# DeepLearnPhysics/u-resnet

Measured on AMD Instinct MI355X. Metric: fwd+bwd images/sec on 3D 192^3x1 U-ResNet, higher is better.
Workload: dtype f32

## Files before the change

### u-resnet_amd/csrc/conv_tiled.hip

```cpp
#include <stdlib.h>

#include "conv_tiled_kernel.h"
#include "wgrad_tiled_kernel.h"

int twgradq_dispatch(const TWPlan& p, const TWgradArgs& a, hipStream_t s);
int twgrad4_dispatch_3d(const TWPlan& p, const TWgradArgs& a, hipStream_t s);
int twgrad4_dispatch_2d(const TWPlan& p, const TWgradArgs& a, hipStream_t s);
int twgradz_dispatch(const TWPlan& p, const TWgradArgs& a, hipStream_t s);

static bool tiled_shape_ok(int cin, int cout, int mode) {
  if (cin % 4 || cout % 4 || cin < 4 || cout < 4) return false;
  if ((cin == 8 || cin == 16) && (cout == 8 || cout == 16)) return true;
  if (mode == 3) return (cin == 8 && cout == 4) || (cin == 4 && cout == 8);
  return (cin == 32 && cout == 16) || (cin == 16 && cout == 32) || (cin == 16 && cout == 4) || (cin == 4 && cout == 16) ||
         (cin == 4 && cout == 8);
}

static bool tiled_disabled() {
  static int v = -1;
  if (v < 0) { const char* e = getenv("URSN_DISABLE_TILED"); v = (e && e[0] == '1') ? 1 : 0; }
  return v == 1;
}

struct Blocking {
// ... 372 lines not shown
      URSN_TRY(launch_reduce_accum_blocked(dw + (size_t)8 * bi * 8, (const float*)scratch, taps, 8, 8, (int64_t)d.cin * 8,
                                           8, nslab, s));
    }
    return 0;
  }
  if (!blocked && use_wgrad4(d, p)) {
    a.x = x;
    a.dz = dy;
    URSN_TRY(p.mode == 3 ? twgrad4_dispatch_3d(p, a, s) : twgrad4_dispatch_2d(p, a, s));
    return launch_reduce_accum(dw, (const float*)scratch, (int64_t)taps * d.cin * d.cout, p.grid, s);
  }
  for (int bi = 0; bi < b.nbi; ++bi)
    for (int bo = 0; bo < b.nbo; ++bo) {
      a.x = x + 16 * bi;
      a.dz = dy + 16 * bo;
      URSN_TRY(p.mode == 3 ? twgrad_dispatch_3d(p, a, s) : twgrad_dispatch_2d(p, a, s));
      if (!blocked) return launch_reduce_accum(dw, (const float*)scratch, (int64_t)taps * d.cin * d.cout, p.grid, s);
      URSN_TRY(launch_reduce_accum_blocked(dw + (size_t)16 * bi * d.cout + 16 * bo, (const float*)scratch, taps, 16, 16,
                                           (int64_t)d.cin * d.cout, d.cout, p.grid, s));
    }
  ursn_relabel_kernel("twgrad<16,16>xB");
  return 0;
}
```

### u-resnet_amd/csrc/elementwise.hip

```cpp
#include "ursn_common.h"

typedef float f32x4 __attribute__((ext_vector_type(4)));

static int next_pow2(int x) { int p = 1; while (p < x) p <<= 1; return p; }

template <int VEC> struct VT;
template <> struct VT<1> { typedef float T; };
template <> struct VT<4> { typedef f32x4 T; };

#ifndef URSN_EW_NT
#define URSN_EW_NT 1
#endif
#ifndef URSN_EW_U
#define URSN_EW_U 2
#endif
#ifndef URSN_EW_ACT_U
#define URSN_EW_ACT_U 4
#endif
template <int VEC> __device__ inline typename VT<VEC>::T ldv(const float* p) {
#if URSN_EW_NT & 1
  return __builtin_nontemporal_load((const typename VT<VEC>::T*)p);
#else
  return *(const typename VT<VEC>::T*)p;
#endif
// ... 305 lines not shown
}

__global__ __launch_bounds__(256) void bn_bwd_final_kernel(const double* __restrict__ partial, int nblocks, int C,
                                                           int64_t V, double* __restrict__ finals,
                                                           float* __restrict__ dbeta, float* __restrict__ dbeta2, int Cw,
                                                           float* __restrict__ coef, const float* __restrict__ mean,
                                                           const float* __restrict__ rstd, const float* __restrict__ beta) {
  const int c = blockIdx.x;
  double s[3];
  reduce_partials<3>(partial, nblocks, C, c, s);
  if (threadIdx.x != 0) return;
  finals[c] = s[0] / (double)V;
  finals[C + c] = s[1] / (double)V;
  finals[2 * C + c] = s[2] / (double)V;
  if (coef) {
    const float r = rstd[c], mu = mean[c];
    const float mg = (float)finals[c], mgx = (float)finals[C + c];
    coef[c] = r;
    coef[C + c] = -(r * r) * mgx;
    coef[2 * C + c] = -r * mg;
    coef[3 * C + c] = mu;
    coef[4 * C + c] = r;
    coef[5 * C + c] = beta ? beta[c] - mu * r : 0.f;
  }
  if (c >= Cw) return;
  if (dbeta) dbeta[c] += (float)s[0];
  if (dbeta2) dbeta2[c] += (float)s[0];
}

template <int VEC>
__global__ __launch_bounds__(256) void bn_bwd_apply_kernel(BnBwdArgs a, int shift, const double* __restrict__ finals) {
  const int CP = 1 << shift;
  const int VPB = 256 >> shift;
  const int c = (threadIdx.x & (CP - 1)) * VEC;
  const int vr = threadIdx.x >> shift;
  if (c >= a.C) return;
  float mu[VEC], rs[VEC], mu2[VEC], rs2[VEC], mg[VEC], mgx[VEC], mgx2[VEC], be[VEC];
  const bool bmask = VEC == 4 && a.relu && a.mask != nullptr;
  const bool ymask = !bmask && a.relu && a.y != nullptr, zmask = !bmask && a.relu && a.y == nullptr;
  const int lane = threadIdx.x & 63;
#pragma unroll
  for (int j = 0; j < VEC; ++j) {
    mu[j] = a.mean[c + j];
    rs[j] = a.rstd[c + j];
    be[j] = zmask ? a.beta[c + j] - mu[j] * rs[j] : 0.f;
    mu2[j] = a.z2 ? a.mean2[c + j] : 0.f;
// ... 68 lines not shown
  Map m = make_map(a.V, a.C, v4 ? 4 : 1);
  double* partial = (double*)a.scratch;
  double* finals = partial + (size_t)m.grid * 3 * a.C;
  int nblocks = m.grid;
  if (a.pre_partial) {
    partial = const_cast<double*>(a.pre_partial);
    nblocks = a.pre_nblocks;
  } else {
    if (v4) hipLaunchKernelGGL(bn_bwd_reduce_kernel<4>, dim3(m.grid), dim3(256), 0, s, a, m.shift, partial);
    else hipLaunchKernelGGL(bn_bwd_reduce_kernel<1>, dim3(m.grid), dim3(256), 0, s, a, m.shift, partial);
    URSN_HIP(hipGetLastError());
  }
  if (a.coef_out) URSN_REQUIRE(!a.z2 && !a.dres && !a.mask && !(a.relu && a.y), "bn_bwd: apply-on-load coefficients need a single BatchNorm, no residual share and the bn(z) > 0 mask");
  hipLaunchKernelGGL(bn_bwd_final_kernel, dim3(a.C), dim3(256), 0, s, (const double*)partial, nblocks, a.C, a.V, finals,
                     a.dbeta, a.z2 ? a.dbeta2 : nullptr, a.Cw > 0 ? a.Cw : a.C, a.coef_out, a.mean, a.rstd, a.relu ? a.beta : nullptr);
  URSN_HIP(hipGetLastError());
  if (a.coef_out) return 0;
  if (v4) hipLaunchKernelGGL(bn_bwd_apply_kernel<4>, dim3(m.grid), dim3(256), 0, s, a, m.shift, (const double*)finals);
  else hipLaunchKernelGGL(bn_bwd_apply_kernel<1>, dim3(m.grid), dim3(256), 0, s, a, m.shift, (const double*)finals);
  URSN_HIP(hipGetLastError());
  return 0;
}

#define URSN_MAX_CLASS 8
__global__ __launch_bounds__(256) void head_kernel(HeadArgs a, double* __restrict__ partial) {
  const int64_t P = (int64_t)a.n * a.pix;
  double loss = 0.0;
  unsigned int n_ok = 0, n_nz = 0, n_ok_nz = 0;
  float sc[URSN_MAX_CLASS], sh[URSN_MAX_CLASS];
#pragma unroll
  for (int k = 0; k < URSN_MAX_CLASS; ++k) {
    sc[k] = 1.f;
    sh[k] = 0.f;
    if (k < a.ncls && a.mean) {
      sc[k] = a.rstd[k];
      sh[k] = a.beta[k] - a.mean[k] * sc[k];
    }
  }
  const float invn = 1.0f / (float)a.n;
  float bg[4] = {0.f, 0.f, 0.f, 0.f}, bgx[4] = {0.f, 0.f, 0.f, 0.f};
  float mu[4];
#pragma unroll
  for (int k = 0; k < 4; ++k) mu[k] = (k < a.ncls && a.mean) ? a.mean[k] : 0.f;
  for (int64_t p = (int64_t)blockIdx.x * blockDim.x + threadIdx.x; p < P; p += (int64_t)gridDim.x * blockDim.x) {
    float z[URSN_MAX_CLASS];
    float m = -INFINITY;
// ... 293 lines not shown
```

### u-resnet_amd/csrc/net.hip

```cpp
#include <math.h>
#include <stdio.h>
#include <stdlib.h>
#include <string.h>

#include <map>
#include <string>
#include <vector>

#include "ursn_common.h"
#include "net_bf16.h"

int conv_dispatch(const ursn_conv_desc& d, ConvPass pass, const float* in, const float* w, float* out, int accumulate,
                  hipStream_t s);
int wgrad_dispatch(const ursn_conv_desc& d, const float* x, const float* dy, float* dw, void* scratch,
                   size_t scratch_bytes, hipStream_t s);

namespace {

struct Arena {
  char* base = nullptr;
  size_t off = 0;
  void* take(size_t bytes) {
    off = (off + 255) & ~(size_t)255;
    void* p = base ? (void*)(base + off) : nullptr;
// ... 43 lines not shown
  int ldim[8][3];
  int64_t lvox[8];
  std::vector<Layer> layers;
  std::vector<Unit> units;
  std::vector<int> deconv;
  std::vector<Act> deconv_in, deconv_out, cat;
  int conv0 = -1, conv1 = -1, conv2 = -1;
  Act a_data, a_conv0, a_conv1, a_pre1;
  std::vector<int> ginit;
  float *params = nullptr, *grads = nullptr, *adam_m = nullptr, *adam_v = nullptr;
  float* dlog = nullptr;
  float* metrics = nullptr;
  void* red_scratch = nullptr;
  void* red_scratch2 = nullptr;
  void* head_scratch = nullptr;
  void* wg_scratch = nullptr;
  size_t wg_scratch_bytes = 0;
  float* dc_scratch = nullptr;
  double* bs_scratch = nullptr;
  int bs_layer = -1, bs_blocks = 0;
  int bs_C = 8;
  int vdz_layer = -1, vdz_relu = 0, vdz_cs = 0;
  const float* vdz_g = nullptr;
  int64_t adam_t = 0;
  int last_n = 0;
  bool profile = false;
  struct ProfRec { int layer; int pass; const char* kernel; double flops; double bytes; hipEvent_t e0, e1; long l0; int launches; };
  std::vector<ProfRec> prof;
  std::vector<hipEvent_t> ev_pool;
  size_t ev_used = 0;
  hipStream_t s2 = nullptr;
  hipStream_t s2_owned = nullptr;
  struct StepGraph { const float* data; const float* label; const float* weight; int n, seen; hipGraphExec_t exec; };
  std::vector<StepGraph> graphs;
  bool graph_broken = false;
  hipStream_t gstream = nullptr;
  hipEvent_t g_in = nullptr, g_out = nullptr;
  std::vector<hipEvent_t> sync_pool;
  size_t sync_used = 0;
  std::vector<hipEvent_t> fwd_pool;
  size_t fwd_used = 0;
  hipEvent_t s2_done = nullptr;
  std::vector<std::pair<std::string, std::string>> cat_names;
  std::map<std::string, Act> named;
  std::map<std::string, int> named_z;
};
// ... 28 lines not shown
int add_layer(ursn_net* n, Arena& A, const std::string& name, int kind, int k, int s, int ci, int co, int lin, int lout,
              int64_t& poff, int relu = 0) {
  Layer L;
  L.name = "UResNet/" + name;
  L.relu = relu;
  L.kind = kind; L.k = k; L.stride = s; L.cin = ci; L.cout = co; L.lin = lin; L.lout = lout;
  int64_t taps = 1;
  for (int j = 0; j < n->cfg.ndim; ++j) taps *= k;
  L.w_n = taps * ci * co;
  L.w_off = poff; poff += L.w_n;
  L.b_off = poff; poff += co;
  memset(&L.desc, 0, sizeof(L.desc));
  L.desc.ndim = n->cfg.ndim;
  L.desc.n = n->cfg.max_batch;
  for (int j = 0; j < n->cfg.ndim; ++j) L.desc.in_sp[j] = n->ldim[lin][3 - n->cfg.ndim + j];
  L.desc.cin = ci; L.desc.cout = co; L.desc.k = k; L.desc.stride = s; L.desc.transposed = kind;
  L.zcs = (co + 3) & ~3;
  L.desc.out_cstride = L.zcs;
  int64_t e = (int64_t)n->cfg.max_batch * n->lvox[lout] * L.zcs;
  L.z = A.floats(e);
  L.dz = n->cfg.trainable ? A.floats(e) : nullptr;
  L.mean = A.floats(L.zcs);
  L.rstd = A.floats(L.zcs);
  L.coef = n->cfg.trainable ? A.floats(6 * L.zcs) : nullptr;
  n->layers.push_back(L);
  n->named_z[L.name] = (int)n->layers.size() - 1;
  return (int)n->layers.size() - 1;
}

int plan(ursn_net* n, Arena& A) {
  const ursn_config& c = n->cfg;
  URSN_REQUIRE(c.ndim == 2 || c.ndim == 3, "len(dims) must be 3 (H,W,C) or 4 (H,W,D,C)");
  URSN_REQUIRE(c.num_strides >= 1 && c.num_strides <= 5, "num_strides %d out of range [1,5]", c.num_strides);
  URSN_REQUIRE(c.cin >= 1 && c.base_filters >= 1 && c.num_class >= 1 && c.num_class <= 8 && c.max_batch >= 1,
               "bad channel / class / batch configuration");
  const int ns = c.num_strides;
  n->nlev = ns + 1;
  for (int l = 0; l <= ns; ++l) {
    n->lvox[l] = 1;
    for (int j = 0; j < 3; ++j) {
      int lead = 3 - c.ndim;
      if (j < lead) { n->ldim[l][j] = 1; continue; }
      int s0 = c.spatial[j - lead];
      URSN_REQUIRE(s0 > 0 && s0 % (1 << ns) == 0, "spatial size %d not divisible by 2^%d (deconv/skip shapes would differ)", s0, ns);
      n->ldim[l][j] = s0 >> l;
      n->lvox[l] *= n->ldim[l][j];
    }
// ... 463 lines not shown
      if (blocks > 0 && blocks <= 16384 && tiled_conv_supported(u, PASS_DGRAD)) { t = u; n->bs_layer = bs->li; n->bs_blocks = blocks; }
    }
    {
      ProfScope pd(n, s, li, 1, 2.0 * layer_macs(n, L, N), layer_bytes(n, L, N));
      URSN_TRY(conv_dispatch(t, PASS_DGRAD, n->vdz_g, n->params + L.w_off, in.g, acc ? 1 : 0, s));
      pd.done(ursn_last_kernel_name());
    }
    need_dgrad = false;
  }
  hipStream_t ws = s;
  if (n->s2) {
    if (n->sync_used == n->sync_pool.size()) {
      hipEvent_t e;
      URSN_HIP(hipEventCreateWithFlags(&e, hipEventDisableTiming));
      n->sync_pool.push_back(e);
    }
    hipEvent_t e = n->sync_pool[n->sync_used++];
    URSN_HIP(hipEventRecord(e, s));
    URSN_HIP(hipStreamWaitEvent(n->s2, e, 0));
    ws = n->s2;
  }
  {
    ProfScope ps(n, ws, li, 2, 2.0 * layer_macs(n, L, N), layer_bytes(n, L, N));
    URSN_TRY(wgrad_dispatch(d, in.p, L.dz, n->grads + L.w_off, n->wg_scratch, n->wg_scratch_bytes, ws));
    ps.done(ursn_last_kernel_name());
  }
  if (dgrad_done_elsewhere) {
    ProfScope pd(n, s, li, 1, 2.0 * layer_macs(n, L, N), layer_bytes(n, L, N));
    pd.done("(fused into conv1 dgrad)");
  }
  if (need_dgrad) {
    bool acc = take_flag(n, in);
    if (in2) URSN_REQUIRE(take_flag(n, *in2) == acc, "split input: the two halves disagree on gradient initialisation");
    d = bwd_desc(n, li, in, N, in2, fused_sc);
    n->bs_layer = -1;
    static const bool bs_off = getenv("URSN_FUSE_BN_BWD_REDUCE") && getenv("URSN_FUSE_BN_BWD_REDUCE")[0] == '0';
    if (bs && bs->li >= 0 && !bs_off) {
      const Layer& T = n->layers[bs->li];
      ursn_conv_desc t = d;
      t.bs_z = T.z; t.bs_z_cstride = T.zcs; t.bs_mean = T.mean; t.bs_rstd = T.rstd; t.bs_beta = n->params + T.b_off;
      t.bs_relu = bs->relu; t.bs_mask = bs->mask;
      if (bs->li2 >= 0) {
        const Layer& T2 = n->layers[bs->li2];
        t.bs_z2 = T2.z; t.bs_z2_cstride = T2.zcs; t.bs_mean2 = T2.mean; t.bs_rstd2 = T2.rstd;
      }
      t.bs_partial = n->bs_scratch;
      const bool fits = T.cout == 8 && T.zcs == 8 && in.C == 8 && in.cs == 8 && !in2 &&
// ... 3 lines not shown
    }
    ProfScope pd(n, s, li, 1, 2.0 * layer_macs(n, L, N), layer_bytes(n, L, N));
    if (n->dc_scratch && deep_conv_supported(d, PASS_DGRAD))
      URSN_TRY(launch_deep_conv(d, PASS_DGRAD, L.dz, n->params + L.w_off, in.g, acc ? 1 : 0, n->dc_scratch, nullptr, 0.f, nullptr, nullptr, s));
    else
      URSN_TRY(conv_dispatch(d, PASS_DGRAD, L.dz, n->params + L.w_off, in.g, acc ? 1 : 0, s));
    pd.done(ursn_last_kernel_name());
  }
  return 0;
}

bool vdz_ok(ursn_net* n, int li, const Act& in, int N, bool two_z_target) {
  static const int mode = getenv("URSN_FUSE_BN_BWD_APPLY") ? atoi(getenv("URSN_FUSE_BN_BWD_APPLY")) : 1;
  const bool off = mode == 0 || (mode == 1 && two_z_target);
  const Layer& L = n->layers[li];
  if (off || n->cfg.ndim != 3 || L.kind || L.k != 3 || L.stride != 1 || L.cin != 8 || L.cout != 8 || L.zcs != 8 || in.C != 8 || in.cs != 8 || !in.g)
    return false;
  ursn_conv_desc d = L.desc;
  d.n = N; d.in_cstride = in.cs; d.out_cstride = L.zcs;
  d.vdz_z = L.z; d.vdz_coef = L.coef; d.vdz_out = L.dz;
  return tiled_conv_supported(d, PASS_DGRAD) != 0;
}

int bn_back(ursn_net* n, int li, const float* dy, int dycs, const float* y, int ycs, int relu, int li2, float* dres,
            int drescs, int dres_acc, int N, hipStream_t s, const unsigned long long* mask = nullptr, const Act* fuse_in = nullptr,
            bool fuse_two_z = false) {
  Layer& L = n->layers[li];
  BnBwdArgs a;
  memset(&a, 0, sizeof(a));
  a.dy = dy; a.dycs = dycs; a.y = mask ? nullptr : y; a.ycs = ycs; a.mask = mask;
  a.z = L.z; a.zcs = L.zcs; a.mean = L.mean; a.rstd = L.rstd; a.dz = L.dz; a.dzcs = L.zcs;
  a.dbeta = n->grads + L.b_off;
  a.beta = n->params + L.b_off;
  if (li2 >= 0) {
    Layer& L2 = n->layers[li2];
    a.z2 = L2.z; a.z2cs = L2.cout; a.mean2 = L2.mean; a.rstd2 = L2.rstd; a.dz2 = L2.dz; a.dz2cs = L2.cout;
    a.dbeta2 = n->grads + L2.b_off;
  }
  a.dres = dres; a.drescs = drescs; a.dres_accumulate = dres_acc;
  a.V = (int64_t)N * n->lvox[L.lout]; a.C = L.cout; a.relu = relu; a.scratch = n->red_scratch;
  if (L.zcs != L.cout && li2 < 0 && !relu && dycs == L.zcs && !dres) { a.C = L.zcs; a.Cw = L.cout; }
  if (n->bs_layer == li && a.C == n->bs_C) { a.pre_partial = n->bs_scratch; a.pre_nblocks = n->bs_blocks; }
  n->bs_layer = -1;
  n->bs_C = 8;
  n->vdz_layer = -1;
  if (fuse_in && li2 < 0 && !dres && !mask && !y && dycs == L.zcs && vdz_ok(n, li, *fuse_in, N, fuse_two_z)) {
    a.coef_out = L.coef;
    n->vdz_layer = li; n->vdz_relu = relu; n->vdz_g = dy; n->vdz_cs = dycs;
  }
  ProfScope ps(n, s, li, 5, 0.0, 4.0 * a.V * a.C * (2.0 * (2 + (relu && !mask) + (li2 >= 0)) + 1 + (li2 >= 0) + (dres != nullptr)));
  URSN_TRY(launch_bn_bwd(a, s));
  ps.done("bn_bwd");
  return 0;
}

int unit_bwd(ursn_net* n, Unit& u, int N, hipStream_t s, const BsTarget* in_target = nullptr) {
  if (u.sc >= 0) {
    URSN_TRY(bn_back(n, u.c2, u.out.g, u.out.cs, u.out.p, u.out.cs, 1, u.sc, nullptr, 0, 0, N, s, u.jmask));
  } else {
    bool acc = take_flag(n, u.in);
    URSN_TRY(bn_back(n, u.c2, u.out.g, u.out.cs, u.out.p, u.out.cs, 1, -1, u.in.g, u.in.cs, acc ? 1 : 0, N, s, u.jmask));
  }
  BsTarget t1;
  t1.li = u.c1;
  if (u.a1_virtual) {
    Act z1 = u.a1;
    z1.p = n->layers[u.c1].z; z1.cs = n->layers[u.c1].zcs;
    URSN_TRY(conv_bwd(n, u.c2, z1, true, N, s, nullptr, -1, false, u.c1, &t1));
  } else {
    URSN_TRY(conv_bwd(n, u.c2, u.a1, true, N, s, nullptr, -1, false, -1, &t1));
  }
  URSN_TRY(bn_back(n, u.c1, u.a1.g, u.a1.cs, nullptr, 0, 0, -1, nullptr, 0, 0, N, s, nullptr, (u.in2.C || u.sc >= 0) ? nullptr : &u.in,
                   in_target && in_target->li2 >= 0));
// ... 34 lines not shown
    if (u.jmask) { t.li = u.c2; t.li2 = u.sc; t.relu = 2; t.mask = u.jmask; }
    return t;
  };
  auto act_of = [&](int li) { BsTarget t; t.li = li; t.relu = 1; return t; };
  tc = join_of(n->units[ui - 1]);
  URSN_TRY(conv_bwd(n, n->conv1, n->a_pre1, true, N, s, nullptr, -1, false, -1, &tc));
  for (int i = ns - 1; i >= 0; --i) {
    tc = join_of(n->units[ui - 2]);
    URSN_TRY(unit_bwd(n, n->units[--ui], N, s, &tc));
    tc = act_of(n->deconv[i]);
    URSN_TRY(unit_bwd(n, n->units[--ui], N, s, &tc));
    const Act& dout = n->deconv_out[i];
    URSN_TRY(bn_back(n, n->deconv[i], dout.g, dout.cs, nullptr, 0, 1, -1, nullptr, 0, 0, N, s));
    tc = join_of(n->units[ui - 1]);
    URSN_TRY(conv_bwd(n, n->deconv[i], n->deconv_in[i], true, N, s, nullptr, -1, false, -1, &tc));
  }
  for (int step = ns - 1; step >= 0; --step) {
    tc = join_of(n->units[ui - 2]);
    URSN_TRY(unit_bwd(n, n->units[--ui], N, s, &tc));
    tc = ui >= 2 ? join_of(n->units[ui - 2]) : act_of(n->conv0);
    URSN_TRY(unit_bwd(n, n->units[--ui], N, s, &tc));
  }
  const Act& a0 = n->a_conv0;
  URSN_TRY(bn_back(n, n->conv0, a0.g, a0.cs, nullptr, 0, 1, -1, nullptr, 0, 0, N, s));
  Act din = n->a_data;
  din.p = const_cast<float*>(data);
  URSN_TRY(conv_bwd(n, n->conv0, din, false, N, s));
  if (n->s2) {
    URSN_HIP(hipEventRecord(n->s2_done, n->s2));
    URSN_HIP(hipStreamWaitEvent(s, n->s2_done, 0));
  }
  return 0;
}

int read_metrics(ursn_net* n, float* out, int cnt, hipStream_t s) {
  float h[4];
  URSN_HIP(hipMemcpyAsync(h, n->metrics, sizeof(h), hipMemcpyDeviceToHost, s));
  URSN_HIP(hipStreamSynchronize(s));
  if (cnt == 3) { out[0] = h[0]; out[1] = h[1]; out[2] = h[2]; }
  else { out[0] = h[1]; out[1] = h[2]; }
  return 0;
}

int check_call(ursn_net* n, const float* data, int N) {
  URSN_REQUIRE(n, "null handle");
  URSN_REQUIRE(data, "input_data is null");
  URSN_REQUIRE(N >= 1 && N <= n->cfg.max_batch, "batch %d outside [1,%d]", N, n->cfg.max_batch);
  return 0;
}
// ... 320 lines not shown
  std::string s(name);
  bool want_z = false, want_g = false, want_dz = false, want_mean = false, want_rstd = false;
  auto strip = [&](const char* suf, bool& f) {
    size_t L = strlen(suf);
    if (s.size() > L && s.compare(s.size() - L, L, suf) == 0) { f = true; s = s.substr(0, s.size() - L); }
  };
  strip(":dz", want_dz);
  strip(":z", want_z);
  strip(":grad", want_g);
  strip(":mean", want_mean);
  strip(":rstd", want_rstd);
  if (want_g && s == "logits") {
    URSN_REQUIRE(net->dlog, "tensor: net is not trainable");
    const Layer& L = net->layers[net->conv2];
    *ptr = net->dlog; *voxels = net->lvox[0]; *channels = L.cout; *cstride = L.zcs;
    return 0;
  }
  if (want_z || want_dz || want_mean || want_rstd) {
    auto it = net->named_z.find(s);
    URSN_REQUIRE(it != net->named_z.end(), "tensor: no layer named %s", s.c_str());
    const Layer& L = net->layers[it->second];
    *ptr = want_z ? L.z : want_dz ? L.dz : want_mean ? L.mean : L.rstd;
    URSN_REQUIRE(*ptr, "tensor: %s does not exist (net is not trainable)", name);
    *voxels = (want_mean || want_rstd) ? 0 : net->lvox[L.lout];
    *channels = L.cout;
    *cstride = L.zcs;
    return 0;
  }
  auto it = net->named.find(s);
  URSN_REQUIRE(it != net->named.end(), "tensor: no activation named %s", s.c_str());
  *ptr = want_g ? it->second.g : it->second.p;
  URSN_REQUIRE(*ptr, "tensor: %s is not materialised (normalised on load inside the consuming convolution, URSN_NORM_ON_LOAD=1)", name);
  *voxels = net->lvox[it->second.lvl];
  *channels = it->second.C;
  *cstride = it->second.cs;
  return 0;
}

extern "C" int ursn_profile_enable(ursn_net* net, int32_t on) {
  URSN_REQUIRE(net, "null handle");
  if (net->bf) return bnet_profile_enable(net->bf, on);
  net->profile = on != 0;
  net->prof.clear();
  net->ev_used = 0;
  return 0;
}
// ... 31 lines not shown
```

### u-resnet_amd/csrc/ursn_common.h

```cpp
#pragma once
#include <hip/hip_runtime.h>
#include <stdint.h>
#include <stddef.h>

#include "../../include/uresnet_hip.h"

void ursn_set_error(const char* fmt, ...);
void ursn_note_kernel(const char* name);
void ursn_relabel_kernel(const char* name);
#ifdef __HIPCC__
#ifndef URSN_XCD_REMAP
#define URSN_XCD_REMAP 1
#endif
__device__ __forceinline__ int ursn_xcd_block(int b, int G) {
#if URSN_XCD_REMAP
  const int q = G >> 3, r = G & 7, x = b & 7, i = b >> 3;
  return (x < r ? x * (q + 1) : r * (q + 1) + (x - r) * q) + i;
#else
  return b;
#endif
}

__device__ __forceinline__ void ursn_sacc(float piv, float& s1, float& s2, float v) {
  const float d = v - piv;
// ... 71 lines not shown
enum ConvPass { PASS_FWD = 0, PASS_DGRAD = 1, PASS_WGRAD = 2 };
int build_geoms(const ursn_conv_desc& d, ConvPass pass, GatherGeom* out8);

struct BnStats {
  double* sum;
  float* mean;
  float* rstd;
};

size_t reduce_scratch_bytes(int64_t voxels, int channels, int nsums);
int reduce_nblocks(int64_t voxels, int channels);

int launch_bn_stats(const float* z, int zcs, int64_t V, int C, float eps, float* mean, float* rstd,
                    void* scratch, hipStream_t s);
int launch_bn_stats_final(const double* partial, int nblocks, int C, int PC, int64_t V, float eps, float* mean,
                          float* rstd, hipStream_t s);
int launch_bn_stats_final_blocked(const double* partial, int nblocks, int C, int CB, int PC, size_t blk_stride, int64_t V, float eps,
                                  float* mean, float* rstd, hipStream_t s);
int tiled_conv_supported(const ursn_conv_desc& d, ConvPass pass);
size_t tiled_conv_stats_scratch_doubles(const ursn_conv_desc& d);
int launch_tiled_conv_bn(const ursn_conv_desc& d, const float* in, const float* w, float* out, double* scratch,
                         float eps, float* mean, float* rstd, hipStream_t s);
int tiled_wgrad_supported(const ursn_conv_desc& d);
int tiled_conv_bs_blocks(const ursn_conv_desc& d);
int igemm_conv_supported(const ursn_conv_desc& d, ConvPass pass);
size_t igemm_stats_scratch_doubles(const ursn_conv_desc& d);
int launch_igemm_conv(const ursn_conv_desc& d, ConvPass pass, const float* in, const float* w, float* out,
                      int accumulate, double* stats_partial, float eps, float* mean, float* rstd, hipStream_t s);
int igemm_wgrad_supported(const ursn_conv_desc& d);
size_t igemm_wgrad_scratch_bytes(const ursn_conv_desc& d);
int launch_igemm_wgrad(const ursn_conv_desc& d, const float* x, const float* dy, float* dw, void* scratch,
                       size_t scratch_bytes, hipStream_t s);
int deep_conv_supported(const ursn_conv_desc& d, ConvPass pass);
size_t deep_conv_scratch_floats(const ursn_conv_desc& d, ConvPass pass);
size_t deep_conv_stats_scratch_doubles(const ursn_conv_desc& d);
int launch_deep_conv(const ursn_conv_desc& d, ConvPass pass, const float* in, const float* w, float* out, int accumulate,
                     float* scratch, double* stats_partial, float eps, float* mean, float* rstd, hipStream_t s);
int deep_wgrad_supported(const ursn_conv_desc& d);
size_t deep_wgrad_scratch_bytes(const ursn_conv_desc& d);
int launch_deep_wgrad(const ursn_conv_desc& d, const float* x, const float* dy, float* dw, void* scratch, size_t scratch_bytes,
                      hipStream_t s);
int pointwise_conv_supported(const ursn_conv_desc& d, ConvPass pass, int accumulate);
size_t pointwise_stats_scratch_doubles(const ursn_conv_desc& d);
int launch_pointwise_conv(const ursn_conv_desc& d, ConvPass pass, const float* in, const float* w, float* out,
                          int accumulate, double* stats_partial, float eps, float* mean, float* rstd, hipStream_t s);
int pointwise_wgrad_supported(const ursn_conv_desc& d);
// ... 30 lines not shown
  const float* res; int rescs;
  float* y; int ycs;
  int64_t V; int C; int relu;
  unsigned long long* mask_out;
};
int launch_bn_act(const BnActArgs& a, hipStream_t s);
static inline size_t bn_mask_words(int64_t V, int C) { return (size_t)((V * C + 255) / 256) * 4; }
static inline bool bn_mask_ok(int C) { int q = C / 4; return (C % 4) == 0 && q >= 1 && q <= 64 && (q & (q - 1)) == 0; }

struct BnBwdArgs {
  const float* dy; int dycs; const float* y; int ycs;
  const float* z; int zcs; const float* mean; const float* rstd; float* dz; int dzcs; float* dbeta;
  const float* beta;
  const float* z2; int z2cs; const float* mean2; const float* rstd2; float* dz2; int dz2cs; float* dbeta2;
  float* dres; int drescs; int dres_accumulate;
  int64_t V; int C; int relu;
  void* scratch;
  const unsigned long long* mask;
  const double* pre_partial; int pre_nblocks;
  int Cw;
  float* coef_out;
};
int launch_bn_bwd(const BnBwdArgs& a, hipStream_t s);

struct HeadArgs {
  const float* z; int z_cs; const float* mean; const float* rstd; const float* beta;
  const float* data; int data_cs; const float* label; const float* weight;
  int n; int64_t pix; int ncls;
  float* softmax_out; float* dlogits;
  int dl_cs;
  float* ana_out;
  double* partial;
  float* metrics;
  void* scratch;
  double* bs_partial;
};
size_t head_scratch_bytes(int n, int64_t pix);
int head_blocks(int n, int64_t pix);
int launch_head_final(const double* partial, int nblocks, int n, int64_t pix, float* metrics, hipStream_t s);
int launch_bn_bwd_final(const double* partial, int nblocks, int C, int64_t V, double* finals, float* dbeta, float* dbeta2,
                        int Cw, hipStream_t s, float* coef_out = nullptr, const float* mean = nullptr, const float* rstd = nullptr,
                        const float* beta = nullptr);
int launch_head(const HeadArgs& a, hipStream_t s);

int launch_adam(float* p, const float* g, float* m, float* v, int64_t n, float lr_t, float b1, float b2,
                float eps, hipStream_t s);
// ... 4 lines not shown
```

### u-resnet_amd/csrc/wgrad_tiled_3d.hip

```cpp
#include "wgrad_tiled_kernel.h"

int twgrad_dispatch_3d(const TWPlan& p, const TWgradArgs& a, hipStream_t s) {
  constexpr int MODE = 3;
  URSN_TW(8, 8) URSN_TW(16, 8) URSN_TW(8, 16) URSN_TW(16, 16) URSN_TW(8, 4) URSN_TW(1, 8)
  ursn_set_error("tiled wgrad 3d: no instantiation for %d->%d", p.cin, p.cout);
  return 3;
}
```

### u-resnet_amd/csrc/wgrad_tiled_kernel.h

```cpp
#pragma once
#include <utility>

#include "ursn_common.h"
#include "buffer_stage.h"

typedef float wg_f32x4 __attribute__((ext_vector_type(4)));

struct TWgradArgs {
  const float* x;
  const float* dz;
  float* slab;
  int N, Z, Y, X;
  int x_cs, dz_cs;
  int zseg, nzseg, nty, ntx;
  int cout_w;
  const float* aff_mean;
  const float* aff_rstd;
  const float* aff_beta;
};

template <int MODE> struct WTile;
template <> struct WTile<3> { static constexpr int TX = 32, TY = 8, NTY = 3, NT = 27; };
template <> struct WTile<2> { static constexpr int TX = 256, TY = 1, NTY = 1, NT = 9; };

template <int... Is, class F>
__device__ __forceinline__ void wg_static_for_impl(std::integer_sequence<int, Is...>, F&& f) {
  (f(std::integral_constant<int, Is>{}), ...);
}
template <int N, class F>
__device__ __forceinline__ void wg_static_for(F&& f) {
  wg_static_for_impl(std::make_integer_sequence<int, N>{}, static_cast<F&&>(f));
}

template <int CIN, int COUT, int MODE>
__global__ __launch_bounds__(256, 1) void twgrad_kernel(TWgradArgs a) {
  using TL = WTile<MODE>;
  constexpr int TX = TL::TX, TY = TL::TY, NTY = TL::NTY, NT = TL::NT;
  constexpr int PX = TX + 2, PY = TY + (NTY == 3 ? 2 : 0), PS = PX * PY;
  constexpr int MT = CIN >= 16 ? CIN / 16 : 1;
  constexpr int NA = CIN >= 16 ? NT * MT : (CIN == 1 ? (NT + 15) / 16 : (NT + 1) / 2);
  constexpr int CT = (COUT + 15) / 16;
  constexpr int XQ = CIN >= 4 ? CIN / 4 : 1, DQ = COUT / 4;
  constexpr int NSX = (XQ * PS + 255) / 256;
  constexpr int NSD = (DQ * TX * TY + 255) / 256;
  constexpr int XPLANE = PS * CIN, DPLANE = TX * TY * COUT;
  constexpr int GPR = TX / 4 / (MODE == 3 ? 1 : 4);
  extern __shared__ __attribute__((aligned(16))) float wlds[];
  float* xr = wlds;
  float* dr = wlds + 4 * XPLANE;

  const int tid = threadIdx.x, lane = tid & 63, wave = tid >> 6;
  const int il = lane & 15, kl = lane >> 4;
  int bid = ursn_xcd_block(blockIdx.x, gridDim.x);
  const int xt = bid % a.ntx; bid /= a.ntx;
  const int yt = bid % a.nty; bid /= a.nty;
  const int zs = bid % a.nzseg;
  const int n = bid / a.nzseg;
  const int x0 = xt * TX, y0 = yt * TY;
// ... 14 lines not shown
    a_off[m] = (tyy * PX + txx) * CIN + ci;
  }
  const int wrow = (MODE == 3) ? 2 * wave : 0;
  const int wcol = (MODE == 3) ? 0 : 64 * wave;
  const int a_lane = ((wrow * PX) + wcol + kl) * CIN;
  const int b_lane = ((wrow * TX) + wcol + kl) * COUT + il;

  wg_f32x4 acc[NA][CT];
#pragma unroll
  for (int m = 0; m < NA; ++m)
#pragma unroll
    for (int c = 0; c < CT; ++c) acc[m][c] = (wg_f32x4){0.f, 0.f, 0.f, 0.f};

  __shared__ wg_f32x4 aff_s[XQ], aff_t[XQ];
  const bool aff = a.aff_mean != nullptr && CIN >= 4;
  if (aff) {
    if (tid < CIN) {
      const float r = a.aff_rstd[tid];
      ((float*)aff_s)[tid] = r;
      ((float*)aff_t)[tid] = a.aff_beta[tid] - a.aff_mean[tid] * r;
    }
    __syncthreads();
  }
  wg_f32x4 sx[NSX], sd[NSD];
  unsigned sx_inb = 0;
  unsigned xgo[NSX], dgo[NSD], xin_mask = 0;
#pragma unroll
  for (int i = 0; i < NSX; ++i) {
    const int idx = tid + i * 256;
    const int s = idx / XQ, q = idx - s * XQ;
    const int yy = s / PX, xx = s - yy * PX;
    const int py = y0 + yy - (NTY == 3 ? 1 : 0), px = x0 + xx - 1;
    const bool ok = idx < XQ * PS && py >= 0 && py < a.Y && px >= 0 && px < a.X;
    xgo[i] = ok ? (unsigned)((py * a.X + px) * a.x_cs + 4 * q) * 4u : URSN_OOB_OFFSET;
    if (ok) xin_mask |= 1u << i;
    asm volatile("" : "+v"(xgo[i]));
  }
  asm volatile("" : "+v"(xin_mask));
#pragma unroll
  for (int i = 0; i < NSD; ++i) {
    const int idx = tid + i * 256;
    const int s = idx / DQ, q = idx - s * DQ;
    const int yy = s / TX, xx = s - yy * TX;
    const int py = y0 + yy, px = x0 + xx;
    const bool ok = idx < DQ * TX * TY && py < a.Y && px < a.X;
    dgo[i] = ok ? (unsigned)((py * a.X + px) * a.dz_cs + 4 * q) * 4u : URSN_OOB_OFFSET;
    asm volatile("" : "+v"(dgo[i]));
  }
  const ptrdiff_t xplane_f = (ptrdiff_t)a.Y * a.X * a.x_cs, dplane_f = (ptrdiff_t)a.Y * a.X * a.dz_cs;
  const unsigned xplane_b = (unsigned)xplane_f * 4u, dplane_b = (unsigned)dplane_f * 4u;
  const float* ximg = a.x + (size_t)n * a.Z * xplane_f;
  const float* dimg = a.dz + (size_t)n * a.Z * dplane_f;
  auto load_x = [&](int zin) {
    const bool zok = zin >= 0 && zin < a.Z;
    sx_inb = zok ? xin_mask : 0u;
    const __amdgpu_buffer_rsrc_t r = ursn_plane_rsrc(ximg + (ptrdiff_t)zin * xplane_f, zok ? xplane_b : 0u);
#pragma unroll
    for (int i = 0; i < NSX; ++i) {
      if constexpr (CIN == 1) sx[i] = (wg_f32x4){ursn_buffer_load_f1(r, xgo[i]), 0.f, 0.f, 0.f};
      else sx[i] = ursn_buffer_load_f4(r, xgo[i]);
    }
  };
  auto store_x = [&](int slot) {
#pragma unroll
    for (int i = 0; i < NSX; ++i) {
      int idx = tid + i * 256;
      if (idx < XQ * PS) {
        if (CIN == 1) xr[(size_t)slot * XPLANE + idx] = sx[i][0];
        else {
          wg_f32x4 v = sx[i];
          if (aff && ((sx_inb >> i) & 1u)) { const int q = idx % XQ; v = v * aff_s[q] + aff_t[q]; }
          *(wg_f32x4*)(xr + (size_t)slot * XPLANE + idx * 4) = v;
        }
      }
    }
  };
  auto load_d = [&](int zin) {
    const bool zok = zin < z1;
    const __amdgpu_buffer_rsrc_t r = ursn_plane_rsrc(dimg + (ptrdiff_t)zin * dplane_f, zok ? dplane_b : 0u);
#pragma unroll
    for (int i = 0; i < NSD; ++i) sd[i] = ursn_buffer_load_f4(r, dgo[i]);
  };
  auto store_d = [&](int slot) {
#pragma unroll
    for (int i = 0; i < NSD; ++i) {
      int idx = tid + i * 256;
      if (idx < DQ * TX * TY) *(wg_f32x4*)(dr + (size_t)slot * DPLANE + idx * 4) = sd[i];
    }
  };

  for (int p = -1; p <= 1; ++p) {
    load_x(z0 + p);
    store_x((z0 + p) & 3);
  }
  load_d(z0);
  store_d(z0 & 1);
  __syncthreads();

  for (int z = z0; z < z1; ++z) {
    load_x(z + 2);
    load_d(z + 1);
    int abase[NA];
#pragma unroll
    for (int m = 0; m < NA; ++m) {
      int tz = a_tz[m] < 0 ? 0 : a_tz[m];
      abase[m] = ((z - 1 + tz) & 3) * XPLANE + a_lane + a_off[m];
    }
    const float* dcur = dr + (size_t)(z & 1) * DPLANE + b_lane;
    wg_static_for<16>([&](auto G) {
      constexpr int g = decltype(G)::value;
// ... 28 lines not shown
#pragma unroll
      for (int r = 0; r < 4; ++r) {
        int row = 4 * kl + r;
        int tap, ci;
        if (CIN >= 16) { tap = m / MT; ci = (m % MT) * 16 + row; }
        else if (CIN == 1) { tap = 16 * m + row; ci = 0; }
        else { tap = 2 * m + (row >> 3); ci = row & 7; }
        if (tap < NT && col < a.cout_w) part[(tap * CIN + ci) * a.cout_w + col] = acc[m][c][r];
      }
    }
  __syncthreads();
  float* slab = a.slab + (size_t)blockIdx.x * (size_t)nred;
  for (int i = tid; i < nred; i += 256)
    slab[i] = ((wlds[i] + wlds[nred + i]) + wlds[2 * nred + i]) + wlds[3 * nred + i];
}

struct TWPlan {
  int mode, cin, cout;
  int Z, Y, X, zseg, nzseg, nty, ntx;
  size_t lds;
  int grid;
};

template <int CIN, int COUT, int MODE>
static int launch_tw(const TWPlan& p, const TWgradArgs& a, hipStream_t s) {
  auto kern = twgrad_kernel<CIN, COUT, MODE>;
  static size_t attr_lds = 48 * 1024;
  if (p.lds > attr_lds) {
    URSN_HIP(hipFuncSetAttribute((const void*)kern, hipFuncAttributeMaxDynamicSharedMemorySize, (int)p.lds));
    attr_lds = p.lds;
  }
  hipLaunchKernelGGL(kern, dim3(p.grid), dim3(256), p.lds, s, a);
  URSN_HIP(hipGetLastError());
  return 0;
}

#define URSN_TW(ci, co)                              \
  if (p.cin == ci && p.cout == co) {                 \
    ursn_note_kernel("twgrad<" #ci "," #co ">");     \
    return launch_tw<ci, co, MODE>(p, a, s);         \
  }

int twgrad_dispatch_3d(const TWPlan& p, const TWgradArgs& a, hipStream_t s);
int twgrad_dispatch_2d(const TWPlan& p, const TWgradArgs& a, hipStream_t s);
```

Measured before the change: 67.94.

## Fuse conv0 BatchNorm-backward apply into the tiled weight-gradient load

```diff
diff --git a/u-resnet_amd/csrc/conv_tiled.hip b/u-resnet_amd/csrc/conv_tiled.hip
--- a/u-resnet_amd/csrc/conv_tiled.hip
+++ b/u-resnet_amd/csrc/conv_tiled.hip
@@ -1,4 +1,5 @@
 #include <stdlib.h>
+#include <string.h>
 
 #include "conv_tiled_kernel.h"
 #include "wgrad_tiled_kernel.h"
@@ -418,3 +419,31 @@
   ursn_relabel_kernel("twgrad<16,16>xB");
   return 0;
 }
+
+int tiled_wgrad_apply_supported(const ursn_conv_desc& d) {
+  TWPlan p;
+  Blocking b;
+  const int ics = d.in_cstride > 0 ? d.in_cstride : d.cin, ocs = d.out_cstride > 0 ? d.out_cstride : d.cout;
+  return d.ndim == 3 && d.cin == 1 && d.cout == 8 && ics == 1 && ocs == 8 && !d.in_mean && !d.in_split && !d.transposed &&
+         make_wplan(d, p, b) && b.nbi == 1 && b.nbo == 1 && p.mode == 3 && p.cin == 1 && p.cout == 8;
+}
+
+int launch_tiled_wgrad_apply(const ursn_conv_desc& d, const float* x, const float* g, const float* z, const float* coef, int relu,
+                             float* dw, void* scratch, size_t scratch_bytes, hipStream_t s) {
+  TWPlan p;
+  Blocking b;
+  URSN_REQUIRE(tiled_wgrad_apply_supported(d) && make_wplan(d, p, b), "tiled wgrad: apply on load not supported for this shape");
+  URSN_REQUIRE(x && g && z && coef && dw, "tiled wgrad: apply on load needs x, g, z and the coefficients");
+  const size_t need = tiled_wgrad_scratch_bytes(d);
+  URSN_REQUIRE(scratch && scratch_bytes >= need, "tiled wgrad: scratch too small (%zu < %zu)", scratch_bytes, need);
+  TWgradArgs a;
+  memset(&a, 0, sizeof(a));
+  a.x = x; a.dz = g; a.slab = (float*)scratch;
+  a.N = d.n; a.Z = p.Z; a.Y = p.Y; a.X = p.X;
+  a.x_cs = 1; a.dz_cs = 8;
+  a.zseg = p.zseg; a.nzseg = p.nzseg; a.nty = p.nty; a.ntx = p.ntx;
+  a.cout_w = 8;
+  a.dz_z = z; a.dz_coef = coef; a.dz_relu = relu;
+  URSN_TRY(twgrad_apply_dispatch_3d(p, a, s));
+  return launch_reduce_accum(dw, (const float*)scratch, (int64_t)27 * 8, p.grid, s);
+}
diff --git a/u-resnet_amd/csrc/elementwise.hip b/u-resnet_amd/csrc/elementwise.hip
--- a/u-resnet_amd/csrc/elementwise.hip
+++ b/u-resnet_amd/csrc/elementwise.hip
@@ -351,6 +351,8 @@
     coef[3 * C + c] = mu;
     coef[4 * C + c] = r;
     coef[5 * C + c] = beta ? beta[c] - mu * r : 0.f;
+    coef[6 * C + c] = mg;
+    coef[7 * C + c] = mgx;
   }
   if (c >= Cw) return;
   if (dbeta) dbeta[c] += (float)s[0];
@@ -465,6 +467,31 @@
   return 0;
 }
 
+__global__ __launch_bounds__(256) void bn_bwd_coef_apply_kernel(const float* __restrict__ g, int gcs, const float* __restrict__ z,
+                                                                 int zcs, const float* __restrict__ coef, int C, int relu,
+                                                                 float* __restrict__ dz, int dzcs, int64_t V) {
+  const int64_t n = V * C;
+  for (int64_t i = (int64_t)blockIdx.x * 256 + threadIdx.x; i < n; i += (int64_t)gridDim.x * 256) {
+    const int64_t v = i / C;
+    const int c = (int)(i - v * C);
+    const float zv = z[v * zcs + c], rs = coef[c], mu = coef[3 * C + c], be = coef[5 * C + c];
+    const float mg = coef[6 * C + c], mgx = coef[7 * C + c];
+    float gj = g[v * gcs + c];
+    const float xh = (zv - mu) * rs;
+    if (relu && !(fmaf(zv, rs, be) > 0.f)) gj = 0.f;
+    dz[v * dzcs + c] = rs * (gj - mg - xh * mgx);
+  }
+}
+
+int launch_bn_bwd_coef_apply(const float* g, int gcs, const float* z, int zcs, const float* coef, int C, int relu, float* dz,
+                             int dzcs, int64_t V, hipStream_t s) {
+  const int64_t n = V * C;
+  const int grid = (int)std::min<int64_t>((n + 255) / 256, 65536);
+  hipLaunchKernelGGL(bn_bwd_coef_apply_kernel, dim3(grid), dim3(256), 0, s, g, gcs, z, zcs, coef, C, relu, dz, dzcs, V);
+  URSN_HIP(hipGetLastError());
+  return 0;
+}
+
 #define URSN_MAX_CLASS 8
 __global__ __launch_bounds__(256) void head_kernel(HeadArgs a, double* __restrict__ partial) {
   const int64_t P = (int64_t)a.n * a.pix;
diff --git a/u-resnet_amd/csrc/net.hip b/u-resnet_amd/csrc/net.hip
--- a/u-resnet_amd/csrc/net.hip
+++ b/u-resnet_amd/csrc/net.hip
@@ -89,6 +89,10 @@
   int bs_C = 8;
   int vdz_layer = -1, vdz_relu = 0, vdz_cs = 0;
   const float* vdz_g = nullptr;
+  int wdz_layer = -1, wdz_relu = 0;
+  const float* wdz_g = nullptr;
+  bool dz0_virtual = false;
+  int dz0_n = 0;
   int64_t adam_t = 0;
   int last_n = 0;
   bool profile = false;
@@ -163,7 +167,7 @@
   L.dz = n->cfg.trainable ? A.floats(e) : nullptr;
   L.mean = A.floats(L.zcs);
   L.rstd = A.floats(L.zcs);
-  L.coef = n->cfg.trainable ? A.floats(6 * L.zcs) : nullptr;
+  L.coef = n->cfg.trainable ? A.floats(8 * L.zcs) : nullptr;
   n->layers.push_back(L);
   n->named_z[L.name] = (int)n->layers.size() - 1;
   return (int)n->layers.size() - 1;
@@ -673,7 +677,12 @@
   }
   {
     ProfScope ps(n, ws, li, 2, 2.0 * layer_macs(n, L, N), layer_bytes(n, L, N));
-    URSN_TRY(wgrad_dispatch(d, in.p, L.dz, n->grads + L.w_off, n->wg_scratch, n->wg_scratch_bytes, ws));
+    if (n->wdz_layer == li)
+      URSN_TRY(launch_tiled_wgrad_apply(d, in.p, n->wdz_g, L.z, L.coef, n->wdz_relu, n->grads + L.w_off, n->wg_scratch,
+                                        n->wg_scratch_bytes, ws));
+    else
+      URSN_TRY(wgrad_dispatch(d, in.p, L.dz, n->grads + L.w_off, n->wg_scratch, n->wg_scratch_bytes, ws));
+    n->wdz_layer = -1;
     ps.done(ursn_last_kernel_name());
   }
   if (dgrad_done_elsewhere) {
@@ -723,9 +732,20 @@
   return tiled_conv_supported(d, PASS_DGRAD) != 0;
 }
 
+bool wdz0_ok(ursn_net* n, const Act& in, int N) {
+  static const bool off = getenv("URSN_CONV0_BN_BWD_IN_WGRAD") && getenv("URSN_CONV0_BN_BWD_IN_WGRAD")[0] == '0';
+  const Layer& L = n->layers[n->conv0];
+  const Act& a0 = n->a_conv0;
+  if (off || !n->cfg.trainable || n->cfg.ndim != 3 || L.cin != 1 || L.cout != 8 || L.zcs != 8 || !L.coef || a0.C != 8 || a0.cs != 8 ||
+      !a0.g || in.cs != 1)
+    return false;
+  ursn_conv_desc d = bwd_desc(n, n->conv0, in, N, nullptr, -1);
+  return tiled_wgrad_apply_supported(d) != 0;
+}
+
 int bn_back(ursn_net* n, int li, const float* dy, int dycs, const float* y, int ycs, int relu, int li2, float* dres,
             int drescs, int dres_acc, int N, hipStream_t s, const unsigned long long* mask = nullptr, const Act* fuse_in = nullptr,
-            bool fuse_two_z = false) {
+            bool fuse_two_z = false, bool apply_in_wgrad = false) {
   Layer& L = n->layers[li];
   BnBwdArgs a;
   memset(&a, 0, sizeof(a));
@@ -745,11 +765,19 @@
   n->bs_layer = -1;
   n->bs_C = 8;
   n->vdz_layer = -1;
-  if (fuse_in && li2 < 0 && !dres && !mask && !y && dycs == L.zcs && vdz_ok(n, li, *fuse_in, N, fuse_two_z)) {
+  n->wdz_layer = -1;
+  if (apply_in_wgrad) {
+    URSN_REQUIRE(li2 < 0 && !dres && !mask && !y && dycs == L.zcs && L.zcs == 8, "BatchNorm-backward apply in the weight gradient: %s", L.name.c_str());
+    a.coef_out = L.coef;
+    n->wdz_layer = li; n->wdz_relu = relu; n->wdz_g = dy;
+  }
+  if (!apply_in_wgrad && fuse_in && li2 < 0 && !dres && !mask && !y && dycs == L.zcs && vdz_ok(n, li, *fuse_in, N, fuse_two_z)) {
     a.coef_out = L.coef;
     n->vdz_layer = li; n->vdz_relu = relu; n->vdz_g = dy; n->vdz_cs = dycs;
   }
-  ProfScope ps(n, s, li, 5, 0.0, 4.0 * a.V * a.C * (2.0 * (2 + (relu && !mask) + (li2 >= 0)) + 1 + (li2 >= 0) + (dres != nullptr)));
+  const double bn_bytes = apply_in_wgrad ? (a.pre_partial ? 0.0 : 4.0 * a.V * a.C * 2.0)
+                                         : 4.0 * a.V * a.C * (2.0 * (2 + (relu && !mask) + (li2 >= 0)) + 1 + (li2 >= 0) + (dres != nullptr));
+  ProfScope ps(n, s, li, 5, 0.0, bn_bytes);
   URSN_TRY(launch_bn_bwd(a, s));
   ps.done("bn_bwd");
   return 0;
@@ -830,9 +858,11 @@
     URSN_TRY(unit_bwd(n, n->units[--ui], N, s, &tc));
   }
   const Act& a0 = n->a_conv0;
-  URSN_TRY(bn_back(n, n->conv0, a0.g, a0.cs, nullptr, 0, 1, -1, nullptr, 0, 0, N, s));
   Act din = n->a_data;
   din.p = const_cast<float*>(data);
+  n->dz0_virtual = wdz0_ok(n, din, N);
+  n->dz0_n = N;
+  URSN_TRY(bn_back(n, n->conv0, a0.g, a0.cs, nullptr, 0, 1, -1, nullptr, 0, 0, N, s, nullptr, nullptr, false, n->dz0_virtual));
   URSN_TRY(conv_bwd(n, n->conv0, din, false, N, s));
   if (n->s2) {
     URSN_HIP(hipEventRecord(n->s2_done, n->s2));
@@ -1199,6 +1229,12 @@
     const Layer& L = net->layers[it->second];
     *ptr = want_z ? L.z : want_dz ? L.dz : want_mean ? L.mean : L.rstd;
     URSN_REQUIRE(*ptr, "tensor: %s does not exist (net is not trainable)", name);
+    if (want_dz && it->second == net->conv0 && net->dz0_virtual) {
+      const Act& a0 = net->a_conv0;
+      URSN_HIP(hipDeviceSynchronize());
+      URSN_TRY(launch_bn_bwd_coef_apply(a0.g, a0.cs, L.z, L.zcs, L.coef, L.zcs, 1, L.dz, L.zcs, (int64_t)net->dz0_n * net->lvox[L.lout], nullptr));
+      URSN_HIP(hipDeviceSynchronize());
+    }
     *voxels = (want_mean || want_rstd) ? 0 : net->lvox[L.lout];
     *channels = L.cout;
     *cstride = L.zcs;
diff --git a/u-resnet_amd/csrc/ursn_common.h b/u-resnet_amd/csrc/ursn_common.h
--- a/u-resnet_amd/csrc/ursn_common.h
+++ b/u-resnet_amd/csrc/ursn_common.h
@@ -117,6 +117,9 @@
 int launch_tiled_conv_bn(const ursn_conv_desc& d, const float* in, const float* w, float* out, double* scratch,
                          float eps, float* mean, float* rstd, hipStream_t s);
 int tiled_wgrad_supported(const ursn_conv_desc& d);
+int tiled_wgrad_apply_supported(const ursn_conv_desc& d);
+int launch_tiled_wgrad_apply(const ursn_conv_desc& d, const float* x, const float* g, const float* z, const float* coef, int relu,
+                             float* dw, void* scratch, size_t scratch_bytes, hipStream_t s);
 int tiled_conv_bs_blocks(const ursn_conv_desc& d);
 int igemm_conv_supported(const ursn_conv_desc& d, ConvPass pass);
 size_t igemm_stats_scratch_doubles(const ursn_conv_desc& d);
@@ -193,6 +196,8 @@
   float* coef_out;
 };
 int launch_bn_bwd(const BnBwdArgs& a, hipStream_t s);
+int launch_bn_bwd_coef_apply(const float* g, int gcs, const float* z, int zcs, const float* coef, int C, int relu, float* dz,
+                             int dzcs, int64_t V, hipStream_t s);
 
 struct HeadArgs {
   const float* z; int z_cs; const float* mean; const float* rstd; const float* beta;
diff --git a/u-resnet_amd/csrc/wgrad_tiled_3d.hip b/u-resnet_amd/csrc/wgrad_tiled_3d.hip
--- a/u-resnet_amd/csrc/wgrad_tiled_3d.hip
+++ b/u-resnet_amd/csrc/wgrad_tiled_3d.hip
@@ -6,3 +6,9 @@
   ursn_set_error("tiled wgrad 3d: no instantiation for %d->%d", p.cin, p.cout);
   return 3;
 }
+
+int twgrad_apply_dispatch_3d(const TWPlan& p, const TWgradArgs& a, hipStream_t s) {
+  URSN_REQUIRE(p.cin == 1 && p.cout == 8 && a.dz_coef && a.dz_z, "tiled wgrad 3d: apply on load needs 1 -> 8 and its coefficients");
+  ursn_note_kernel("twgrad<1,8>+bn_bwd");
+  return launch_tw<1, 8, 3, true>(p, a, s);
+}
diff --git a/u-resnet_amd/csrc/wgrad_tiled_kernel.h b/u-resnet_amd/csrc/wgrad_tiled_kernel.h
--- a/u-resnet_amd/csrc/wgrad_tiled_kernel.h
+++ b/u-resnet_amd/csrc/wgrad_tiled_kernel.h
@@ -17,6 +17,9 @@
   const float* aff_mean;
   const float* aff_rstd;
   const float* aff_beta;
+  const float* dz_z;
+  const float* dz_coef;
+  int dz_relu;
 };
 
 template <int MODE> struct WTile;
@@ -32,8 +35,9 @@
   wg_static_for_impl(std::make_integer_sequence<int, N>{}, static_cast<F&&>(f));
 }
 
-template <int CIN, int COUT, int MODE>
+template <int CIN, int COUT, int MODE, bool DZL = false>
 __global__ __launch_bounds__(256, 1) void twgrad_kernel(TWgradArgs a) {
+  static_assert(!DZL || COUT == 8, "apply on load: 8-channel dz");
   using TL = WTile<MODE>;
   constexpr int TX = TL::TX, TY = TL::TY, NTY = TL::NTY, NT = TL::NT;
   constexpr int PX = TX + 2, PY = TY + (NTY == 3 ? 2 : 0), PS = PX * PY;
@@ -94,7 +98,8 @@
     }
     __syncthreads();
   }
-  wg_f32x4 sx[NSX], sd[NSD];
+  wg_f32x4 sx[NSX], sd[NSD], sz[DZL ? NSD : 1];
+  unsigned din_mask = 0, sd_inb = 0;
   unsigned sx_inb = 0;
   unsigned xgo[NSX], dgo[NSD], xin_mask = 0;
 #pragma unroll
@@ -117,12 +122,22 @@
     const int py = y0 + yy, px = x0 + xx;
     const bool ok = idx < DQ * TX * TY && py < a.Y && px < a.X;
     dgo[i] = ok ? (unsigned)((py * a.X + px) * a.dz_cs + 4 * q) * 4u : URSN_OOB_OFFSET;
+    if (ok) din_mask |= 1u << i;
     asm volatile("" : "+v"(dgo[i]));
+  }
+  static_assert(256 % DQ == 0, "staging: fixed channel quad per thread");
+  float cf[DZL ? 8 : 1][4];
+  if constexpr (DZL) {
+#pragma unroll
+    for (int k = 0; k < 8; ++k)
+#pragma unroll
+      for (int j = 0; j < 4; ++j) cf[k][j] = a.dz_coef[k * 8 + 4 * (tid % DQ) + j];
   }
   const ptrdiff_t xplane_f = (ptrdiff_t)a.Y * a.X * a.x_cs, dplane_f = (ptrdiff_t)a.Y * a.X * a.dz_cs;
   const unsigned xplane_b = (unsigned)xplane_f * 4u, dplane_b = (unsigned)dplane_f * 4u;
   const float* ximg = a.x + (size_t)n * a.Z * xplane_f;
   const float* dimg = a.dz + (size_t)n * a.Z * dplane_f;
+  const float* zimg = DZL ? a.dz_z + (size_t)n * a.Z * dplane_f : nullptr;
   auto load_x = [&](int zin) {
     const bool zok = zin >= 0 && zin < a.Z;
     sx_inb = zok ? xin_mask : 0u;
@@ -152,12 +167,34 @@
     const __amdgpu_buffer_rsrc_t r = ursn_plane_rsrc(dimg + (ptrdiff_t)zin * dplane_f, zok ? dplane_b : 0u);
 #pragma unroll
     for (int i = 0; i < NSD; ++i) sd[i] = ursn_buffer_load_f4(r, dgo[i]);
+    if constexpr (DZL) {
+      sd_inb = zok ? din_mask : 0u;
+      const __amdgpu_buffer_rsrc_t rz = ursn_plane_rsrc(zimg + (ptrdiff_t)zin * dplane_f, zok ? dplane_b : 0u);
+#pragma unroll
+      for (int i = 0; i < NSD; ++i) sz[i] = ursn_buffer_load_f4(rz, dgo[i]);
+    }
   };
   auto store_d = [&](int slot) {
 #pragma unroll
     for (int i = 0; i < NSD; ++i) {
       int idx = tid + i * 256;
-      if (idx < DQ * TX * TY) *(wg_f32x4*)(dr + (size_t)slot * DPLANE + idx * 4) = sd[i];
+      if (idx < DQ * TX * TY) {
+        wg_f32x4 v = sd[i];
+        if constexpr (DZL) {
+          const wg_f32x4 g = sd[i], zv = sz[i];
+          v = (wg_f32x4){0.f, 0.f, 0.f, 0.f};
+          if ((sd_inb >> i) & 1u) {
+#pragma unroll
+            for (int j = 0; j < 4; ++j) {
+              float gj = g[j];
+              const float rs = cf[0][j], xh = (zv[j] - cf[3][j]) * rs;
+              if (a.dz_relu && !(fmaf(zv[j], rs, cf[5][j]) > 0.f)) gj = 0.f;
+              v[j] = rs * (gj - cf[6][j] - xh * cf[7][j]);
+            }
+          }
+        }
+        *(wg_f32x4*)(dr + (size_t)slot * DPLANE + idx * 4) = v;
+      }
     }
   };
 
@@ -232,9 +269,9 @@
   int grid;
 };
 
-template <int CIN, int COUT, int MODE>
+template <int CIN, int COUT, int MODE, bool DZL = false>
 static int launch_tw(const TWPlan& p, const TWgradArgs& a, hipStream_t s) {
-  auto kern = twgrad_kernel<CIN, COUT, MODE>;
+  auto kern = twgrad_kernel<CIN, COUT, MODE, DZL>;
   static size_t attr_lds = 48 * 1024;
   if (p.lds > attr_lds) {
     URSN_HIP(hipFuncSetAttribute((const void*)kern, hipFuncAttributeMaxDynamicSharedMemorySize, (int)p.lds));
@@ -253,3 +290,4 @@
 
 int twgrad_dispatch_3d(const TWPlan& p, const TWgradArgs& a, hipStream_t s);
 int twgrad_dispatch_2d(const TWPlan& p, const TWgradArgs& a, hipStream_t s);
+int twgrad_apply_dispatch_3d(const TWPlan& p, const TWgradArgs& a, hipStream_t s);
```

New measurement: 68.48, median of 6. About the same (+0.8%).
